# sjtuyinjie/Ground-Fusion2

Hardware: AMD Instinct MI355X
Metric: sliding-window solves/sec (10-kf, 2k landmarks) (higher is better)
Workload: dtype f64; 1 GPU; BASELINE configs[1]: 10-keyframe VI-wheel window, 2000 landmarks (K=9457 visual factors avg), marginalisation prior n=86, full optimization() = <=8 dogleg iterations + re-anchor + MARGIN_OLD; windows_per_gpu=8192, unique_windows=8, parallelism=windows sharded over 1 rank(s), no collective

## Files before the change

ground-fusion2_amd/csrc/gfbe_kernels.hip:

```cpp
#include "gfbe_devutil.h"
#include "gfbe_factors.h"
#include "gfbe_gnss_item.h"
#include <type_traits>

namespace gfd {

#ifndef GFBE_ASM_U
#define GFBE_ASM_U 4
#endif
#if GFBE_DIAG
#define ASM_TP_ON(d) (!(d).asm_legacy)
#else
#define ASM_TP_ON(d) true
#endif
#ifndef GFBE_KVIS_WAVES
#define GFBE_KVIS_WAVES 3
#endif
#ifndef GFBE_KVIS_STAMP
#define GFBE_KVIS_STAMP 0
#endif

#define PREP_WSYNC() do { __threadfence_block(); __builtin_amdgcn_wave_barrier(); } while (0)
template <int n>
__device__ __forceinline__ int sqrt_info_from_cov_wave(const double *cov, double *lu, double *inv, double *U, const int lane) {
// ... 594 lines not shown
          if (MODE != 1) {
            Hll += vc[u][1];
            gl += vc[u][2];
            if (YM) {
#pragma unroll
              for (int q = 0; q < 3; q++) Dsum[q] += vc[u][3 + q];
            } else {
#pragma unroll
              for (int q = 0; q < 6; q++) { hC[q] += vc[u][3 + q]; if (FULL) hC[6 + q] += vc[u][9 + q]; }
              if (FULL) hC[12] += vc[u][15];
            }
          }
        }
      }
    }
#undef VC_LD
    asm volatile("" :: "v"(cost));
    LSTAMP_ANY(18);
  }
  if (YM) {
#pragma unroll
    for (int q = 0; q < 3; q++) { hC[q] = Dsum[q]; hC[3 + q] = yx[q]; }
  }
  if (MODE == 0 && d.spec && tile == 0 && lane == 0) d.ctl[w].sw_mu[SPEC ? 1 - c.lb : c.lb] = SPEC ? mu_after_accept(c.mu) : c.mu;
  if (MODE == 0 && valid) {
    const bool first = !SPEC && c.iter == 0;
    const double mu_w = SPEC ? mu_after_accept(c.mu) : c.mu;
    double sl = 1.0, sw = 0.0;
    if (m > 0 && !is_const) {
      sl = first ? (d.opt.jacobi_scaling ? 1.0 / (1.0 + sqrt(Hll)) : 1.0) : d.lm_sl[slot];
      const double hs2 = sl * sl * Hll;
      sw = sqrt(sl * sl / (hs2 + mu_w * clamp_diag(hs2)));
    }
    if (first) d.lm_sl[slot] = sl;
    d.lm_sw[slot] = sw;
  }
  if (MODE != 1 && valid) {
    d.lm_Hll[slot] = Hll;
    d.lm_gl[slot] = gl;
#pragma unroll
    for (int q = 0; q < NHC; q++) d.lm_hC[(size_t)q * TL + slot] = hC[q];
  }
  KSTAMP(30);
  LSTAMP_ANY(19);
  cost = wave_sum(cost);
  if (lane == 0) {
    if (CAND) d.tile_cand[((size_t)w * d.max_tiles + tile) * 4] = cost;
    else d.tile_cost[(size_t)w * d.max_tiles + tile] = cost;
  }
}

__device__ __forceinline__ double candidate_tile(const BatchDev &d, const WinDesc &ds, const WinCtl &c, const int w, const int tile, const int t);
template <int MODE, bool FULL, bool SPEC = false>
__global__ __launch_bounds__(LM_TILE, (MODE == 0 && !FULL) ? GFBE_KVIS_WAVES : 2) void k_vis(BatchDev d0, int write_records) {
  const BatchDev d = MODE == 0 ? lin_view(d0, SPEC ? 1 - d0.ctl[blockIdx.x].lb : d0.ctl[blockIdx.x].lb) : d0;
  vis_body<MODE, FULL, 1, SPEC>(d, (MODE == 1 || SPEC) ? 0 : write_records, blockIdx.x, blockIdx.y, 0, (MODE == 1 || SPEC) && write_records);
}

#ifndef VIS_CHUNK
#define VIS_CHUNK 4
#endif
template <bool SPEC>
__global__ __launch_bounds__(LM_TILE, GFBE_KVIS_WAVES) void k_vis_chunk(BatchDev d0, int head_in, int nsub) {
  const int w = blockIdx.x;
  const WinCtl &c = d0.ctl[w];
  if (!SPEC && (c.done || c.reuse)) return;
  if (SPEC && (c.done || !c.have_step)) return;
  const int lbw = SPEC ? 1 - c.lb : c.lb;
  const BatchDev d = lin_view(d0, lbw);
  const WinDesc &ds = d.desc[w];
  const int sframe = blockIdx.y / nsub, sub = blockIdx.y - sframe * nsub;
  const int t0 = ds.sf_tile_begin[sframe] + VIS_CHUNK * sub, t1 = min(t0 + VIS_CHUNK, ds.sf_tile_begin[sframe + 1]);
  if (t0 >= t1) return;
  const int cur = c.cur, buf = SPEC ? 1 - cur : cur;
  const double *X = d.x + ((size_t)w * 2 + buf) * NA;
  const bool chead = SPEC && head_in;
  const double c1 = c.c1, c2 = c.c2;
  const bool first = !SPEC && c.iter == 0;
  const double mu_w = SPEC ? mu_after_accept(c.mu) : c.mu;
  const double sq = d.opt.vis_sqrt_info, delta = d.opt.huber_delta;
  const int jac_scale = d.opt.jacobi_scaling;
  const int lm_off_c = ds.lm_off;
  constexpr int XLD = 17;
  __shared__ PairConstY pcs[NF];
  __shared__ FrameConst fcs;
  __shared__ double xs[LM_TILE * XLD];
  const int lane = threadIdx.x;
  const size_t TL = d.tot_lm;
  int p_info;
  double p_pt[3], p_lam, p_sl = 0.0, p_vl = 0.0, p_yl = 0.0, p_ob[2];
#define VC_PREFETCH(TILE)                                                                                           \
  {                                                                                                                  \
    const int slot_ = lm_off_c + (TILE) * LM_TILE + lane;                                                            \
    p_info = d.lm_info[slot_];                                                                                       \
    _Pragma("unroll") for (int q = 0; q < 3; q++) p_pt[q] = d.lm_pts[(size_t)q * TL + slot_];                        \
    p_lam = d.lam[(size_t)(chead ? cur : buf) * TL + slot_];                                                         \
    if (chead) { p_sl = d.lm_sl[slot_]; p_vl = d.lm_vl[slot_]; p_yl = d.lm_yl[slot_]; }                              \
    p_ob[0] = d.lm_obs[slot_]; p_ob[1] = d.lm_obs[TL + slot_];                                                       \
  }
  VC_PREFETCH(t0)
  const double td = X[A_TD];
  {
    const double *src = d.pc + (((size_t)w * 3 + buf) * NPAIR + sframe * NF) * PC_DOUBLES;
    static_assert(PCY_DOUBLES <= LM_TILE && FC_DOUBLES <= LM_TILE, "one lane per entry of a pair record");
    const int ql = min(lane, (int)PCY_DOUBLES - 1);
    double rec[NF - 1];
#pragma unroll
    for (int jj = 0; jj < NF - 1; jj++) rec[jj] = src[(size_t)min(sframe + 1 + jj, NF - 1) * PC_DOUBLES + ql];
    const double fcv = src[(size_t)sframe * PC_DOUBLES + min(lane, (int)FC_DOUBLES - 1)];
#pragma unroll
    for (int jj = 0; jj < NF - 1; jj++) if (sframe + 1 + jj < NF && lane < (int)PCY_DOUBLES) ((double *)&pcs[min(sframe + 1 + jj, NF - 1)])[lane] = rec[jj];
    if (lane < (int)FC_DOUBLES) ((double *)&fcs)[lane] = fcv;
  }
  __syncthreads();
  for (int tile = t0; tile < t1; tile++) {
    const int slot = lm_off_c + tile * LM_TILE + lane;
    const int info = p_info;
    const double pix = p_pt[0], piy = p_pt[1], piz = p_pt[2];
    double lam = p_lam;
    const double c_sl = p_sl, c_vl = p_vl, c_yl = p_yl;
    double nob[2] = {p_ob[0], p_ob[1]};
    if (tile + 1 < t1) VC_PREFETCH(tile + 1)
    const bool valid = (info >> 24) & 1;
    const int m = valid ? ((info >> 8) & 0xff) : 0;
    const bool is_const = (info >> 16) & 1;
    int mmax = m;
#pragma unroll
    for (int o = 32; o > 0; o >>= 1) mmax = max(mmax, __shfl_xor(mmax, o, 64));
    double cost = 0.0;
    if (chead) {
      double d2, n2;
      lam = candidate_lm(lam, c_sl, c_vl, c_yl, c1, c2, valid && !is_const && m > 0, d2, n2);
      d.lam[(size_t)(1 - cur) * TL + slot] = lam;
      d2 = wave_sum(d2); n2 = wave_sum(n2);
      if (lane == 0) {
        double *o = d.tile_cand + ((size_t)w * d.max_tiles + tile) * 4;
        o[1] = d2; o[2] = n2;
      }
    }
    double Hll = 0.0, gl = 0.0, Dsum[3] = {0.0, 0.0, 0.0};
    const double yinv_l = 1.0 / lam;
    const double ycx = pix * yinv_l, ycy = piy * yinv_l, ycz = piz * yinv_l;
    vec3 yf, ye, yx;
#pragma unroll
    for (int a = 0; a < 3; a++) {
      yf[a] = __builtin_fma(fcs.W(a, 0), ycx, __builtin_fma(fcs.W(a, 1), ycy, fcs.W(a, 2) * ycz));
      ye[a] = yf[a] + fcs.wt[a];
      yx[a] = ye[a] + fcs.dPc[a];
    }
    double *xr = xs + lane * XLD;
    xr[7] = 0.0; xr[15] = 0.0;
    for (int k = 0; k < mmax; k++) {
      double r[2], Jl[2], hp[3];
      const double pjx = nob[0], pjy = nob[1];
      if (k + 1 < mmax) {
        const double *ob = d.lm_obs + (size_t)(k + 1) * 5 * TL + slot;
        nob[0] = ob[0]; nob[1] = ob[TL];
      }
      if (k < m) {
        double g0[3], g1[3];
        const double ck = visual_lin_y(pcs[sframe + 1 + k], ycx, ycy, ycz, yf, yinv_l, td, pjx, pjy, 0.0, 0.0, td, sq, delta, r, g0, g1, Jl);
        cost += ck;
        const vec3 y0 = cross3(mk3(g0[0], g0[1], g0[2]), yx), y1 = cross3(mk3(g1[0], g1[1], g1[2]), yx);
        const double w0 = is_const ? 0.0 : Jl[0], w1 = is_const ? 0.0 : Jl[1];
        vec3 dv;
#pragma unroll
        for (int q = 0; q < 3; q++) dv[q] = __builtin_fma(g0[q], w0, g1[q] * w1);
        Hll += __builtin_fma(w0, w0, w1 * w1);
        gl += __builtin_fma(w0, r[0], w1 * r[1]);
#pragma unroll
        for (int q = 0; q < 3; q++) Dsum[q] += dv[q];
#pragma unroll
        for (int q = 0; q < 3; q++) hp[q] = dv[q];
#pragma unroll
        for (int q = 0; q < 3; q++) { xr[q] = g0[q]; xr[3 + q] = y0[q]; xr[8 + q] = g1[q]; xr[11 + q] = y1[q]; }
        xr[6] = r[0]; xr[14] = r[1];
      } else {
#pragma unroll
        for (int q = 0; q < 7; q++) { xr[q] = 0.0; xr[8 + q] = 0.0; }
      }
#pragma unroll
      for (int q = 0; q < 2; q++) asm volatile("" : "+v"(nob[q]));
      if (k < m) {
#pragma unroll
        for (int q = 0; q < 3; q++) d.lm_hP[((size_t)k * 6 + q) * TL + slot] = hp[q];
      }
      typedef double dbl4_y __attribute__((ext_vector_type(4)));
      dbl4_y acc0 = {0, 0, 0, 0};
      const int lr = lane & 15, lk = lane >> 4;
      __threadfence_block();
      __builtin_amdgcn_wave_barrier();
#pragma unroll
      for (int blk = 0; blk < LM_TILE / 4 / 8; blk++) {
        double va[8];
#pragma unroll
        for (int u = 0; u < 8; u++) va[u] = xs[(4 * (8 * blk + u) + lk) * XLD + lr];
#pragma unroll
        for (int u = 0; u < 8; u++) acc0 = __builtin_amdgcn_mfma_f64_16x16x4f64(va[u], va[u], acc0, 0, 0, 0);
      }
      __builtin_amdgcn_wave_barrier();
      const double s0 = acc0[0] + __shfl_down(acc0[2], 8, 64), s1 = acc0[1] + __shfl_down(acc0[3], 8, 64);
      double *vo = d.vis_part + (((size_t)w * d.max_tiles + tile) * MAXOBS + k) * VPY_STRIDE;
      if (lr < 7) {
        { const int a = lk; if (a <= lr) vo[7 * a - a * (a - 1) / 2 + lr - a] = s0; }
        { const int a = lk + 4; if (a <= lr) vo[7 * a - a * (a - 1) / 2 + lr - a] = s1; }
      }
      __builtin_amdgcn_wave_barrier();
    }
    if (d.spec && tile == 0 && lane == 0) d.ctl[w].sw_mu[lbw] = mu_w;
    if (valid) {
      double sl = 1.0, sw = 0.0;
      if (m > 0 && !is_const) {
        sl = first ? (jac_scale ? 1.0 / (1.0 + sqrt(Hll)) : 1.0) : (chead ? c_sl : d.lm_sl[slot]);
        const double hs2 = sl * sl * Hll;
        sw = sqrt(sl * sl / (hs2 + mu_w * clamp_diag(hs2)));
      }
      if (first) d.lm_sl[slot] = sl;
      d.lm_sw[slot] = sw;
      d.lm_Hll[slot] = Hll;
      d.lm_gl[slot] = gl;
#pragma unroll
      for (int q = 0; q < 3; q++) { d.lm_hC[(size_t)q * TL + slot] = Dsum[q]; d.lm_hC[(size_t)(3 + q) * TL + slot] = yx[q]; }
    }
    cost = wave_sum(cost);
    if (lane == 0) {
      if (SPEC) d.tile_cand[((size_t)w * d.max_tiles + tile) * 4] = cost;
      else d.tile_cost[(size_t)w * d.max_tiles + tile] = cost;
    }
  }
#undef VC_PREFETCH
}

template <int MODE, bool FULL>
__global__ __launch_bounds__(LM_TILE, 1) void k_vis_split(BatchDev d, int write_records) {
  vis_body<MODE, FULL, LIN_SMALL_KS>(d, write_records, blockIdx.x, blockIdx.y / LIN_SMALL_KS, blockIdx.y % LIN_SMALL_KS);
}

template <int MODE>
__global__ __launch_bounds__(256) void k_lio_window(BatchDev d0, int spec) {
  const int w = blockIdx.y, wg = blockIdx.x, t = threadIdx.x;
  const WinDesc &ds = d0.desc[w];
  if (ds.lio_n == 0) return;
  const WinCtl &c = d0.ctl[w];
  if (MODE == 0 && !spec && (c.done || c.reuse)) return;
  if ((MODE == 1 || spec) && (c.done || !c.have_step)) return;
  const BatchDev d = MODE == 0 ? lin_view(d0, spec ? 1 - c.lb : c.lb) : d0;
  const int buf = (MODE == 1 || spec) ? 1 - c.cur : c.cur;
  const double *X = d.x + ((size_t)w * 2 + buf) * NA + A_POSE(ds.lio_frame);
  const vec3 tw = ld3(X);
  const mat3 R = qrot(ldq(X + 3));
  constexpr int NACC = (MODE == 0) ? 28 : 1;
  double acc[NACC];
#pragma unroll
  for (int q = 0; q < NACC; q++) acc[q] = 0.0;
  const double sq = ds.lio_sqrt_info, delta = ds.lio_huber;
  for (int k = wg * 256 + t; k < ds.lio_n; k += LIOW_WGS * 256) {
    const double *f = d.lio + (size_t)(ds.lio_off + k) * 8;
    const vec3 p = ld3(f), nv = ld3(f + 3);
    const double sw = sq * f[7];
    double r = sw * (dot3(nv, add(mv(R, p), tw)) + f[6]);
    double scale = 1.0, cost = 0.5 * r * r;
    if (delta > 0.0) {
      double s1, rs, asn;
      cost = corrector(r * r, delta, &s1, &rs, &asn);
      scale = s1;
    }
    if (MODE == 1) { acc[0] += cost; continue; }
    const vec3 nR = tmv(R, nv);
    double J[6];
    J[0] = sw * nv[0]; J[1] = sw * nv[1]; J[2] = sw * nv[2];
    J[3] = -sw * (nR[1] * p[2] - nR[2] * p[1]); J[4] = -sw * (nR[2] * p[0] - nR[0] * p[2]); J[5] = -sw * (nR[0] * p[1] - nR[1] * p[0]);
#pragma unroll
    for (int a = 0; a < 6; a++) J[a] *= scale;
    r *= scale;
    int e = 0;
#pragma unroll
    for (int a = 0; a < 6; a++)
#pragma unroll
      for (int b = a; b < 6; b++) acc[e++] += J[a] * J[b];
#pragma unroll
    for (int a = 0; a < 6; a++) acc[21 + a] += J[a] * r;
    acc[27] += cost;
  }
  __shared__ double red[4][NACC];
  const int lane = t & 63, wave = t >> 6;
#pragma unroll
  for (int q = 0; q < NACC; q++) {
    double v = acc[q];
#pragma unroll
    for (int o = 32; o > 0; o >>= 1) v += __shfl_xor(v, o, 64);
    if (lane == 0) red[wave][q] = v;
  }
  __syncthreads();
  double *out = d.lio_part + ((size_t)w * LIOW_WGS + wg) * LIOW_PART;
  if (t < NACC) out[MODE == 1 ? 28 : t] = red[0][t] + red[1][t] + red[2][t] + red[3][t];
}

__device__ __forceinline__ void pairsum_body(const BatchDev &d, const int marg, const int w, const int pair) {
  const WinDesc &ds = d.desc[w];
  const WinCtl &c = d.ctl[w];
  if (!marg && (c.done || c.reuse)) return;
  int i = 0, rem = pair;
  while (rem >= NF - 1 - i) { rem -= NF - 1 - i; i++; }
  const int j = i + 1 + rem;
  if (marg && i != 0) return;
  const int p = i * NF + j;
  if (ds.pair_begin[p + 1] == ds.pair_begin[p]) return;
  const double *vp = d.vis_part + (size_t)w * d.max_tiles * MAXOBS * VP_STRIDE + (size_t)(j - i - 1) * VP_STRIDE + threadIdx.x;
  double s = 0.0;
  for (int t = ds.sf_tile_begin[i]; t < ds.sf_tile_begin[i + 1]; t++) {
    if (((d.lm_info[ds.lm_off + t * LM_TILE] >> 8) & 0xff) <= j - i - 1) break;
    if (TILE_OWNED(d, t)) s += vp[(size_t)t * MAXOBS * VP_STRIDE];
  }
  if (marg) d.pair_part[((size_t)w * NF + j) * VP_STRIDE + threadIdx.x] = s;
}
__global__ __launch_bounds__(VP_STRIDE) void k_pairsum(BatchDev d, int marg) { pairsum_body(d, marg, blockIdx.y, blockIdx.x); }

__device__ __forceinline__ bool imu_nz(int r, int c) {
  const int mask[5] = {0x03F, 0x052, 0x09E, 0x108, 0x210};
  return (mask[r / 3] >> (c / 3)) & 1;
}
__device__ __forceinline__ bool wheel_nz(int r, int c) {
  if (c >= 20) return true;
  if (c >= 18) return r < 3;
  return r < 3 || ((c / 3) & 1);
}
__device__ __forceinline__ bool dense_pass_active(const WinCtl &c, int mode, int spec = 0) {
  if (mode == 0 && !spec && (c.done || c.reuse)) return false;
  if ((mode == 1 || spec) && (c.done || !c.have_step)) return false;
  return true;
}
#define RAW_IMU (15 + 15 * 30)
#define RAW_WHEEL (6 + 6 * 22)
__device__ __forceinline__ size_t raw_of(int f, int w, int B, int raw_len) { return ((size_t)f * ((B + 3) >> 2) + (w >> 2)) * raw_len * 4 + (w & 3); }
__global__ __launch_bounds__(64) void k_dense_raw(BatchDev d, int mode, int spec) {
  const int f = blockIdx.x, w = blockIdx.y * 64 + threadIdx.x;
  if (w >= d.B) return;
  const WinDesc &ds = d.desc[w];
  const WinCtl &c = d.ctl[w];
  if (!dense_pass_active(c, mode, spec)) return;
  const int buf = (mode == 1 || spec) ? 1 - c.cur : c.cur;
  const double *X = (mode >= 2) ? d.xout + (size_t)w * NA : d.x + ((size_t)w * 2 + buf) * NA;
  const size_t B = d.B;
  if (f < MAX_IMU) {
    if (f >= ds.n_imu) return;
    const int fi = ds.imu_frame[f];
    if (mode >= 2 && !(mode == 2 && fi == 0 && d.imu[ds.imu_off + f].sum_dt < 10.0)) return;
    double *out = d.raw_imu + raw_of(f, w, (int)B, RAW_IMU);
    imu_raw(&d.imu[ds.imu_off + f], d.opt.g_norm, X + A_POSE(fi), X + A_SB(fi), X + A_POSE(fi + 1), X + A_SB(fi + 1), out,
            mode == 1 ? nullptr : out + 15 * 4, 4);
  } else {
// ... 482 lines not shown
  } else {
    dense_body<true>(d, VM, 0, w, y - ny_tiles, SPEC, lsm);
  }
#if GFBE_LIN_STAMP
  if (MODE == GFBE_LIN_STAMP_MODE && (threadIdx.x & 63) == 0) {
    const int f = y - ny_tiles;
    const int kind = tile_wg ? 1 : (f < MAX_IMU ? 2 : (f < MAX_IMU + MAX_WHEEL ? 3 : (f == MAX_IMU + MAX_WHEEL ? 4 : 5)));
    atomicMax(ls + kind, (unsigned long long)wall_clock64());
    if (tile_wg && y == 0) ls[6] = wall_clock64();
    if (tile_wg && y == ny_tiles - 1) ls[7] = wall_clock64();
    if (threadIdx.x == 0 && f == MAX_IMU) ls[11] = wall_clock64();
  }
#endif
  if ((MODE == 1 || SPEC) && (fuse & 4)) {
    if (!tile_wg) { __syncthreads(); if (threadIdx.x >= 64) return; }
    WinCtl &c = d.ctl[w];
    AcceptLocal la;
    la.done = c.done; la.have_step = c.have_step; la.iter = c.iter; la.cur = c.cur; la.num_successful = c.num_successful;
    la.termination = c.termination; la.status = c.status; la.reuse = c.reuse; la.lb = c.lb;
    la.cost = c.cost; la.x_norm = c.x_norm; la.model_change = c.model_change; la.radius = c.radius; la.step_norm = c.step_norm; la.mu = c.mu;
    la.cand_cost = c.cand_cost;
    if (!arrive_last(d.win_cnt + 2 * w + 1, gridDim.y, threadIdx.x)) return;
#if GFBE_LIN_STAMP
    if (MODE == GFBE_LIN_STAMP_MODE && threadIdx.x == 0) ls[12] = wall_clock64();
#endif
    accept_body(d, w, threadIdx.x, la, c, SPEC ? 2 : 1);
    if (threadIdx.x == 0) {
      if (SPEC) c.lb = la.lb;
      c.done = la.done; c.have_step = la.have_step; c.cur = la.cur; c.num_successful = la.num_successful; c.termination = la.termination;
      c.status = la.status; c.reuse = la.reuse; c.cost = la.cost; c.x_norm = la.x_norm; c.radius = la.radius; c.mu = la.mu; c.cand_cost = la.cand_cost;
#if GFBE_LIN_STAMP
      if (MODE == GFBE_LIN_STAMP_MODE) ls[13] = wall_clock64();
#endif
    }
  }
}

typedef double dbl4_t __attribute__((ext_vector_type(4)));
#ifndef HS_LD
#define HS_LD 75
#endif

__device__ __forceinline__ int schur_pair(int I, int J) { return I * 5 - I * (I - 1) / 2 + (J - I); }

__device__ __forceinline__ int schur_group_first(int g, int ng) { return ng >= NF ? g : (g == 0 ? 0 : (g == 1 ? 2 : (g == 2 ? 3 : 6))); }
struct SchurLds {
  double hs[LM_TILE * HS_LD + 8];
  double s_rt[NF][12];
  int s_sf[NF + 1];
};
__device__ __forceinline__ SchurLds &schur_lds() { __shared__ SchurLds s; return s; }
template <bool LEAN>
__device__ __forceinline__ void schur_body(const BatchDev &d, const int marg, const int w, const int grp) {
  const WinDesc &ds = d.desc[w];
  WinCtl &c = d.ctl[w];
  if (!marg && (c.done || c.reuse)) return;
  if (marg && grp != 0) return;
  const int sub = (!marg && d.schur_groups == 2 * NF) ? 2 : 1;
  const int ng = marg ? NF : d.schur_groups / sub, half = grp % sub;
  const int gi = grp / sub;
  const int s_first = schur_group_first(gi, ng), s_end = marg ? 1 : (gi == ng - 1 ? NF : schur_group_first(gi + 1, ng));
  const int tb = ds.sf_tile_begin[s_first], te = ds.sf_tile_begin[s_end];
  const int tfirst = sub == 2 ? tb + half : tb + ((d.rank - tb) % d.world + d.world) % d.world;
  if (tfirst >= te) {
    if (marg) for (int q = threadIdx.x; q < SCHUR_STRIDE; q += 256) d.schur_part[((size_t)w * d.schur_groups) * SCHUR_STRIDE + q] = 0.0;
    return;
  }
  SchurLds &lds_ = schur_lds();
  double *const hs = lds_.hs;
  const size_t TL = d.tot_lm;
  const int t = threadIdx.x, lane = t & 63, wave = t >> 6;
  const bool compact = !marg;
  const int coff = compact ? 1 - 6 * s_first : 0;
  const int I0 = compact ? 0 : (6 * s_first) / 16;
  const int wv = __builtin_amdgcn_readfirstlane(wave);
  const int nside = compact ? (1 + 6 * (NF - s_first) + (d.vis_full ? 7 : 0) + 15) / 16 : 5 - I0, npairs = nside * (nside + 1) / 2;
  int pI[4], pJ[4];
#pragma unroll
  for (int q = 0; q < 4; q++) {
    int idx = 4 * q + wv, I = I0;
    pI[q] = -1; pJ[q] = -1;
    if (idx < npairs) {
      if (compact) { int J = 0; while ((J + 1) * (J + 2) / 2 <= idx) J++; pJ[q] = J; pI[q] = idx - J * (J + 1) / 2; }
      else { while (idx >= 5 - I) { idx -= 5 - I; I++; } pI[q] = I; pJ[q] = I + idx; }
    }
  }
  dbl4_t acc0 = {0.0, 0.0, 0.0, 0.0}, acc1 = acc0, acc2 = acc0, acc3 = acc0;
  const int lr = lane & 15, lk = lane >> 4;
  const int l = t & 63, part = t >> 6;
  const bool spec_sw = !marg && d.spec && c.sw_mu[c.lb] != c.mu;
  const double spec_mu = spec_sw ? c.mu : 0.0;
  const bool hc_full = !LEAN && (marg || d.vis_full);
  int *const s_sf = lds_.s_sf;
  double (*const s_rt)[12] = lds_.s_rt;
  const bool yrows = LEAN || (!marg && !d.vis_full);
  if (t <= NF) s_sf[t] = ds.sf_tile_begin[t];
  if (yrows && t < NF * 12) s_rt[t / 12][t % 12] = d.pc[(((size_t)w * 3 + c.cur) * NPAIR + (t / 12) * (NF + 1)) * PC_DOUBLES + LM_RT_OFF + t % 12];
  const int lm_off_c = ds.lm_off;
  __syncthreads();
  auto sframe_of = [&](int tile) __attribute__((always_inline)) { int sf = s_first; for (int q = s_first + 1; q < s_end; q++) sf += (tile >= s_sf[q]) ? 1 : 0; return sf; };
#define SCHUR_PV 20
#define SCHUR_PV_LEAN 12
#define SCHUR_PREFETCH(PV, PHLL, PSL, PINFO, PS, TILE)                                                                 \
  {                                                                                                                      \
    const int tile_ = min((TILE), te - 1);                                                                               \
    const int slot_ = lm_off_c + tile_ * LM_TILE + l;                                                                    \
    PS = sframe_of(tile_);                                                                                               \
    const int klast_ = max(NF - 2 - PS, 0);                     \
    PINFO = d.lm_info[slot_];                                                                                            \
    PHLL = (marg || spec_sw ? d.lm_Hll : d.lm_sw)[slot_];               \
    if (spec_sw) PSL = d.lm_sl[slot_];                  \
    const double *gl_ = d.lm_gl + slot_;                                                                                 \
     \
     \
    if (LEAN) {                                                                                                          \
      _Pragma("unroll") for (int idx_ = 0; idx_ < SCHUR_PV_LEAN; idx_++) {                                                 \
        const int u_ = max(idx_ - 3, 0) / 3, q_ = max(idx_ - 3, 0) - 3 * u_;                                             \
        const int kk_ = min(part - 1 + 3 * u_, klast_), k9_ = min(9, klast_);                                            \
        const double *src_ = idx_ < 3 ? d.lm_hC + (size_t)(3 + idx_) * TL + slot_                                       \
                           : (part == 0 ? (u_ == 0 ? d.lm_hC + (size_t)q_ * TL + slot_                                  \
                                                   : (u_ == 1 ? gl_ : d.lm_hP + ((size_t)k9_ * 6 + q_) * TL + slot_))   \
                                        : d.lm_hP + ((size_t)kk_ * 6 + q_) * TL + slot_);                                \
        PV[idx_] = *src_;                                                                                                \
      }                                                                                                                  \
    } else                                                                                                               \
    _Pragma("unroll") for (int idx_ = 0; idx_ < SCHUR_PV; idx_++) {                                                      \
      const int u_ = idx_ / 6, q_ = idx_ - 6 * u_;                                                                       \
      const int kk_ = min(part - 1 + 3 * u_, klast_), k9_ = min(9, klast_);                                              \
       \
      const int q9_ = idx_ - HC - 1;                                                                                     \
      const double *src_ = part == 0 ? (idx_ < HC ? d.lm_hC + (size_t)((idx_ < 6 || hc_full) ? idx_ : 5) * TL + slot_   \
                                                  : (idx_ == HC ? gl_ : ((yrows && q9_ >= 3) ? d.lm_hC + (size_t)q9_ * TL + slot_ \
                                                                                             : d.lm_hP + ((size_t)k9_ * 6 + q9_) * TL + slot_))) \
                                     : ((yrows && q_ >= 3) ? d.lm_hC + (size_t)q_ * TL + slot_ : d.lm_hP + ((size_t)kk_ * 6 + q_) * TL + slot_); \
      PV[idx_] = *src_;                                                                                                  \
    }                                                                                                                    \
  }
  const bool stamp_wg = (w == 0 && grp == 0 && t == 0 && !marg);
  double *stamp = d.timing + 8;
  if (stamp_wg) { stamp[0] = (double)wall_clock64(); stamp[5] = (double)clock64(); }
  const int tstep = sub == 2 ? 2 : d.world;
#define SCHUR_SLOT(Q, ACC)                                                                          \
    if (pI[Q] >= 0 && (compact ? pJ[Q] <= jl : ((pI[Q] <= jl || pI[Q] == 4) && (pJ[Q] <= jl || pJ[Q] == 4)))) {   \
      const double *pa = hs + 16 * pI[Q] + lr + lk * HS_LD, *pb = hs + 16 * pJ[Q] + lr + lk * HS_LD; \
      _Pragma("unroll") for (int hf = 0; hf < 2; hf++) {       \
        double va[LM_TILE / 8], vb[LM_TILE / 8];                                                    \
        _Pragma("unroll") for (int kk = 0; kk < LM_TILE / 8; kk++) { va[kk] = pa[4 * (8 * hf + kk) * HS_LD]; vb[kk] = pb[4 * (8 * hf + kk) * HS_LD]; } \
        _Pragma("unroll") for (int kk = 0; kk < LM_TILE / 8; kk++) ACC = __builtin_amdgcn_mfma_f64_16x16x4f64(va[kk], vb[kk], ACC, 0, 0, 0); \
      }                                                                                             \
    }
#define SCHUR_LEAN_SLOT(Q, ACC)                                                                                        \
    if (pI[Q] >= 0 && pJ[Q] <= jl) {                                                                                     \
      const double *pa = hs + 16 * pI[Q] + lr + lk * HS_LD, *pb = hs + 16 * pJ[Q] + lr + lk * HS_LD;                     \
      _Pragma("unroll") for (int c_ = 0; c_ < 4; c_++) if (4 * c_ < nk) {                                                \
        double va[4], vb[4];                                                                                             \
        _Pragma("unroll") for (int kk = 0; kk < 4; kk++) { va[kk] = pa[4 * (4 * c_ + kk) * HS_LD]; vb[kk] = pb[4 * (4 * c_ + kk) * HS_LD]; } \
        _Pragma("unroll") for (int kk = 0; kk < 4; kk++) ACC = __builtin_amdgcn_mfma_f64_16x16x4f64(va[kk], vb[kk], ACC, 0, 0, 0); \
      }                                                                                                                  \
    }
#define SCHUR_RUN_TILE(PV, PHLL, PSL, PINFO, PS, TILE, REFILL)                                                          \
  {                                                                                                                      \
    __syncthreads();                                                                                                     \
    if (stamp_wg && (TILE) == tfirst) stamp[1] = (double)wall_clock64();                                                 \
    const int ps = PS, pm0 = __builtin_amdgcn_readfirstlane(PINFO);                                                      \
    const int jl = __builtin_amdgcn_readfirstlane(compact ? (d.vis_full ? nside - 1 : (6 * (ps - s_first + ((pm0 >> 8) & 0xff) + 1)) >> 4) \
                                                          : (6 * (ps + ((pm0 >> 8) & 0xff) + 1) - 1) >> 4);              \
     \
    const unsigned long long vmask_ = LEAN ? __builtin_amdgcn_ballot_w64((PINFO >> 24) & 1) : ~0ull;                       \
    const int nk = vmask_ ? (64 - __builtin_clzll(vmask_) + 3) >> 2 : 0;                                                 \
    {                                                                                                                    \
      const int s = ps, kmax = NF - 1 - s;                                                  \
      const bool valid = (PINFO >> 24) & 1;                                                                              \
      const int m = (PINFO >> 8) & 0xff;                                                                                 \
      const bool is_const = (PINFO >> 16) & 1;                                                                           \
      double sw = 0.0;                                                                                                   \
      if (valid && m > 0 && (marg || !is_const))                                                                         \
        sw = marg ? sqrt((PHLL > d.opt.marg_eps) ? 1.0 / PHLL : 0.0) : PHLL;                                             \
      if (spec_sw && valid && m > 0 && !is_const) {                    \
        const double hs2_ = PSL * PSL * PHLL;                                                                            \
        sw = sqrt(PSL * PSL / (hs2_ + spec_mu * clamp_diag(hs2_)));                                                      \
      }                                                                                                                  \
      double *row = hs + l * HS_LD + coff;                                                                               \
      if (part == 0) {                                                                                                   \
        for (int q = compact ? 6 * s_first : 16 * I0; q < 6 * s; q++) row[q] = 0.0;                                      \
        double blk0[6];                                                                                                  \
        if (yrows) lm_row_block(s_rt[s], PV + (LEAN ? 3 : 0), PV + (LEAN ? 0 : 3), true, blk0);                      \
        else { _Pragma("unroll") for (int q = 0; q < 6; q++) blk0[q] = PV[q]; }                                          \
        _Pragma("unroll") for (int q = 0; q < 6; q++) { row[6 * s + q] = sw * blk0[q]; row[T_EX + q] = hc_full ? sw * PV[6 + q] : 0.0; } \
        row[T_TD] = hc_full ? sw * PV[12] : 0.0;                                                                         \
        if (compact) {                                                                                                   \
          row[-coff] = sw * PV[LEAN ? 6 : HC];                                                 \
          for (int q = NV + coff; q < min(16 * nside, (int)HS_LD); q++) row[q - coff] = 0.0;      \
        } else {                                                                                                         \
          row[NV] = sw * PV[HC];                                                                                         \
          _Pragma("unroll") for (int q = NV + 1; q < HS_LD; q++) row[q] = 0.0;                                           \
        }                                                                                                                \
        if (9 < kmax) {                                                    \
          const bool written = valid && 9 < m;                                                                           \
          double blk9[6];                                                                                                \
          if (yrows) lm_row_block(s_rt[min(s + 10, NF - 1)], PV + (LEAN ? 9 : HC + 1), PV + (LEAN ? 0 : 3), false, blk9);                       \
          else { _Pragma("unroll") for (int q = 0; q < 6; q++) blk9[q] = PV[HC + 1 + q]; }                               \
          _Pragma("unroll") for (int q = 0; q < 6; q++) row[6 * (s + 10) + q] = written ? sw * blk9[q] : 0.0;            \
        }                                                                                                                \
      } else {                                                                                                           \
        _Pragma("unroll") for (int u = 0; u < 3; u++) {                                                                  \
          const int k = part - 1 + 3 * u;                                                                                \
          if (k < kmax) {                                                                                                \
             \
            const bool written = valid && k < m;                                                                         \
            double blkk[6];                                                                                              \
            if (yrows) lm_row_block(s_rt[s + 1 + k], PV + (LEAN ? 3 + 3 * u : 6 * u), PV + (LEAN ? 0 : 6 * u + 3), false, blkk);     \
            else { _Pragma("unroll") for (int q = 0; q < 6; q++) blkk[q] = PV[u * 6 + q]; }                              \
            _Pragma("unroll") for (int q = 0; q < 6; q++) row[6 * (s + 1 + k) + q] = written ? sw * blkk[q] : 0.0;       \
          }                                                                                                              \
        }                                                                                                                \
      }                                                                                                                  \
    }                                                                                                                    \
    __syncthreads();                                                                                                     \
    if (stamp_wg && (TILE) == tfirst) stamp[2] = (double)wall_clock64();                                                 \
    SCHUR_PREFETCH(PV, PHLL, PSL, PINFO, PS, (REFILL))          \
    if (LEAN) {                                                                                                         \
      SCHUR_LEAN_SLOT(0, acc0) SCHUR_LEAN_SLOT(1, acc1) SCHUR_LEAN_SLOT(2, acc2) SCHUR_LEAN_SLOT(3, acc3)               \
    } else {                                                                                                             \
      SCHUR_SLOT(0, acc0)                                                                                                \
      SCHUR_SLOT(1, acc1)                                                                                                \
      SCHUR_SLOT(2, acc2)                                                                                                \
      SCHUR_SLOT(3, acc3)                                                                                                \
    }                                                                                                                    \
  }
  double preA[SCHUR_PV], aHll = 0.0, aSl = 0.0;
  int aInfo = 0, aS = 0;
  SCHUR_PREFETCH(preA, aHll, aSl, aInfo, aS, tfirst)
  for (int tile = tfirst; tile < te; tile += tstep) SCHUR_RUN_TILE(preA, aHll, aSl, aInfo, aS, tile, tile + tstep)
#undef SCHUR_RUN_TILE
#undef SCHUR_SLOT
#undef SCHUR_LEAN_SLOT
#undef SCHUR_PREFETCH
#undef SCHUR_PV
#undef SCHUR_PV_LEAN
  if (stamp_wg) { stamp[3] = (double)wall_clock64(); stamp[4] = (double)(te - tb); stamp[6] = (double)clock64(); }
  double *out = d.schur_part + ((size_t)w * d.schur_groups + grp) * SCHUR_STRIDE;
#define SCHUR_OUT(Q, ACC)                                                         \
  if (pI[Q] >= 0) {                                                               \
    double *o = out + (size_t)(compact ? pJ[Q] * (pJ[Q] + 1) / 2 + pI[Q] : schur_pair(pI[Q], pJ[Q])) * 256; \
    _Pragma("unroll") for (int r = 0; r < 4; r++) o[(lk + 4 * r) * 16 + lr] = ACC[r]; \
  }
  SCHUR_OUT(0, acc0)
  SCHUR_OUT(1, acc1)
  SCHUR_OUT(2, acc2)
  SCHUR_OUT(3, acc3)
#undef SCHUR_OUT
}
#ifndef GFBE_SCHUR_WGS
#define GFBE_SCHUR_WGS 4
#endif
__global__ __launch_bounds__(256, GFBE_SCHUR_WGS) void k_schur(BatchDev d0, int marg) {
  const BatchDev d = marg ? d0 : lin_view(d0, d0.ctl[blockIdx.x].lb);
  if (!marg && d.schur_groups == SCHUR_GROUPS && !d.vis_full) schur_body<true>(d, 0, blockIdx.x, blockIdx.y);
  else schur_body<false>(d, marg, blockIdx.x, blockIdx.y);
}
#ifndef GFBE_LINSCHUR_WGS
#define GFBE_LINSCHUR_WGS 3
#endif
#define LS_XLD 17
template <bool SPEC>
__global__ __launch_bounds__(256, GFBE_LINSCHUR_WGS) void k_linschur(BatchDev d0, int head_in, int gate_mu) {
  const int w = blockIdx.x;
  const int grp = blockIdx.y == 1 ? 2 : (blockIdx.y == 2 ? 1 : (int)blockIdx.y);
  const WinCtl &c = d0.ctl[w];
  if (c.done) return;
  if (SPEC) { if (!c.have_step) return; }
  else { if (c.reuse) return; if (gate_mu && c.sw_mu[c.lb] == c.mu) return; }
  const int lbw = SPEC ? 1 - c.lb : c.lb;
  const BatchDev d = lin_view(d0, lbw);
  const WinDesc &ds = d.desc[w];
  const int s_first = schur_group_first(grp, SCHUR_GROUPS), s_end = grp == SCHUR_GROUPS - 1 ? (int)NF : schur_group_first(grp + 1, SCHUR_GROUPS);
  const int tb = ds.sf_tile_begin[s_first], te = ds.sf_tile_begin[s_end];
  if (tb >= te) return;
  __shared__ double hs[LM_TILE * HS_LD + 8];
  static_assert(4 * LM_TILE * LS_XLD <= LM_TILE * HS_LD + 8, "the evaluation panels live inside the Schur panel");
  __shared__ double Psum[4][5][LM_TILE];
  __shared__ double Pcost[4];
  __shared__ PairConstY pcs[NF];
  __shared__ FrameConst fcs;
  __shared__ double s_rt[NF][12];
  const int t = threadIdx.x, lane = t & 63, wave = t >> 6;
  const int wv = __builtin_amdgcn_readfirstlane(wave);
  const int rot = __builtin_amdgcn_readfirstlane((int)(((unsigned)w * 0x9E3779B1u) >> 20) + grp);
  const int mr = (wv + rot) & 3;
  const size_t TL = d.tot_lm;
  const int cur = c.cur;
  const int buf = SPEC ? 1 - cur : cur;
  const double *X = d.x + ((size_t)w * 2 + buf) * NA;
  const double *pcw = d.pc + ((size_t)w * 3 + buf) * NPAIR * PC_DOUBLES;
  const bool chead = SPEC && head_in;
  const double c1 = c.c1, c2 = c.c2;
  const bool first = !SPEC && c.iter == 0;
  const double mu_w = SPEC ? mu_after_accept(c.mu) : c.mu;
  const double sq = d.opt.vis_sqrt_info, delta = d.opt.huber_delta;
  const int jac_scale = d.opt.jacobi_scaling;
  const double td = X[A_TD];
  int sfb[NF + 1];
#pragma unroll
  for (int q = 0; q <= NF; q++) sfb[q] = ds.sf_tile_begin[q];
  const int lm_off_c = ds.lm_off;
  if (t < NF * 12) s_rt[t / 12][t % 12] = pcw[(size_t)(t / 12) * (NF + 1) * PC_DOUBLES + LM_RT_OFF + t % 12];
  const int coff = 1 - 6 * s_first;
  const int nside = (1 + 6 * (NF - s_first) + 15) / 16, npairs = nside * (nside + 1) / 2;
  int pI[4], pJ[4];
#pragma unroll
  for (int q = 0; q < 4; q++) {
    const int idx = 4 * q + mr;
    pI[q] = -1; pJ[q] = -1;
    if (idx < npairs) { int J = 0; while ((J + 1) * (J + 2) / 2 <= idx) J++; pJ[q] = J; pI[q] = idx - J * (J + 1) / 2; }
  }
  dbl4_t acc0 = {0.0, 0.0, 0.0, 0.0}, acc1 = acc0, acc2 = acc0, acc3 = acc0;
  const int lr = lane & 15, lk = lane >> 4;
  double *const xs = hs + (size_t)wave * (LM_TILE * LS_XLD);
  int p_info;
  double p_pt[3], p_lam, p_sl = 1.0, p_vl = 0.0, p_yl = 0.0, p_ob[3][2];
#define LS_PREFETCH(TILE)                                                                                           \
  {                                                                                                                  \
    const int er_ = (wv + rot + (TILE)) & 3;                                                                         \
    const int tile_ = min((TILE), te - 1);                                                                           \
    const int slot_ = lm_off_c + tile_ * LM_TILE + lane;                                                             \
    p_info = d.lm_info[slot_];                                                                                       \
    _Pragma("unroll") for (int q = 0; q < 3; q++) p_pt[q] = d.lm_pts[(size_t)q * TL + slot_];                        \
    p_lam = d.lam[(size_t)(chead ? cur : buf) * TL + slot_];                                                         \
    if (chead) { p_vl = d.lm_vl[slot_]; p_yl = d.lm_yl[slot_]; }                                                     \
    if (!first) p_sl = d.lm_sl[slot_];                                                                               \
    _Pragma("unroll") for (int u = 0; u < 3; u++) {                                                                  \
      const int k_ = min(er_ + 4 * u, (int)MAXOBS - 1);                                                              \
      p_ob[u][0] = d.lm_obs[((size_t)k_ * 5 + 0) * TL + slot_];                                                      \
      p_ob[u][1] = d.lm_obs[((size_t)k_ * 5 + 1) * TL + slot_];                                                      \
    }                                                                                                                \
  }
  LS_PREFETCH(tb)
  int cur_sf = -1;
  for (int tile = tb; tile < te; tile++) {
    int sf = s_first;
#pragma unroll
    for (int q = 1; q < NF; q++) sf += (q > s_first && q < s_end && tile >= sfb[q]) ? 1 : 0;
    if (sf != cur_sf) {
      const double *src = pcw + (size_t)sf * NF * PC_DOUBLES;
      for (int e = t; e < (NF - 1 - sf) * (int)PCY_DOUBLES; e += 256) {
        const int j = sf + 1 + e / (int)PCY_DOUBLES, q = e % (int)PCY_DOUBLES;
        ((double *)&pcs[j])[q] = src[(size_t)j * PC_DOUBLES + q];
      }
      if (t < (int)FC_DOUBLES) ((double *)&fcs)[t] = src[(size_t)sf * PC_DOUBLES + t];
      cur_sf = sf;
    }
    __syncthreads();
    const int er = (wv + rot + tile) & 3;
    const int slot = lm_off_c + tile * LM_TILE + lane;
    const int info = p_info;
    const bool valid = (info >> 24) & 1;
    const int m = valid ? ((info >> 8) & 0xff) : 0;
    const bool is_const = (info >> 16) & 1;
    int mmax = m;
#pragma unroll
    for (int o = 32; o > 0; o >>= 1) mmax = max(mmax, __shfl_xor(mmax, o, 64));
    mmax = __builtin_amdgcn_readfirstlane(mmax);
    double lam = p_lam;
    const double sl_old = p_sl;
    if (chead) {
      double d2, n2;
      lam = candidate_lm(lam, sl_old, p_vl, p_yl, c1, c2, valid && !is_const && m > 0, d2, n2);
      if (er == 0) {
        d.lam[(size_t)(1 - cur) * TL + slot] = lam;
        d2 = wave_sum(d2); n2 = wave_sum(n2);
        if (lane == 0) { double *o = d.tile_cand + ((size_t)w * d.max_tiles + tile) * 4; o[1] = d2; o[2] = n2; }
      }
    }
    const double yinv_l = 1.0 / lam;
    const double ycx = p_pt[0] * yinv_l, ycy = p_pt[1] * yinv_l, ycz = p_pt[2] * yinv_l;
    vec3 yf, yx;
#pragma unroll
    for (int a = 0; a < 3; a++) {
      yf[a] = __builtin_fma(fcs.W(a, 0), ycx, __builtin_fma(fcs.W(a, 1), ycy, fcs.W(a, 2) * ycz));
      yx[a] = (yf[a] + fcs.wt[a]) + fcs.dPc[a];
    }
    double *xr = xs + lane * LS_XLD;
    xr[7] = 0.0; xr[15] = 0.0;
    double Hq = 0.0, gq = 0.0, Dq[3] = {0.0, 0.0, 0.0}, cq = 0.0, dk[3][3];
// ... 1938 lines not shown
```

Before: 129,600 solves/s.

## Skip empty MFMA blocks and redundant row zeroing in landmark and Schur kernels

In the landmark linearisation kernel, a wave ballot over active observations sets how many 16-lane groups hold data. The per-observation MFMA outer-product loop only runs over those groups, and the zero-fill is limited to lanes inside them. In the Schur tile builder, a per-16-row chunk bound (jlc) skips MFMA chunks whose column block lies past that chunk's extent. Row zeroing for the pose prefix and the extrinsic/TD/tail columns is done only when the frame index changes or on the first tile, and observation blocks past the tile's minimum count are zeroed instead of being computed. This cuts wasted MFMA and shared-memory traffic on sparse tiles, at the cost of extra branching, a non-unrolled loop, and correctness depending on LDS rows staying valid between tiles.

```diff
diff --git a/ground-fusion2_amd/csrc/gfbe_kernels.hip b/ground-fusion2_amd/csrc/gfbe_kernels.hip
--- a/ground-fusion2_amd/csrc/gfbe_kernels.hip
+++ b/ground-fusion2_amd/csrc/gfbe_kernels.hip
@@ -770,6 +770,8 @@
     xr[7] = 0.0; xr[15] = 0.0;
     for (int k = 0; k < mmax; k++) {
       double r[2], Jl[2], hp[3];
+      const unsigned long long act = __builtin_amdgcn_ballot_w64(k < m);
+      const int ng = act ? (64 - __builtin_clzll(act) + 15) >> 4 : 0;
       const double pjx = nob[0], pjy = nob[1];
       if (k + 1 < mmax) {
         const double *ob = d.lm_obs + (size_t)(k + 1) * 5 * TL + slot;
@@ -793,7 +795,7 @@
 #pragma unroll
         for (int q = 0; q < 3; q++) { xr[q] = g0[q]; xr[3 + q] = y0[q]; xr[8 + q] = g1[q]; xr[11 + q] = y1[q]; }
         xr[6] = r[0]; xr[14] = r[1];
-      } else {
+      } else if (lane < 16 * ng) {
 #pragma unroll
         for (int q = 0; q < 7; q++) { xr[q] = 0.0; xr[8 + q] = 0.0; }
       }
@@ -808,13 +810,13 @@
       const int lr = lane & 15, lk = lane >> 4;
       __threadfence_block();
       __builtin_amdgcn_wave_barrier();
-#pragma unroll
-      for (int blk = 0; blk < LM_TILE / 4 / 8; blk++) {
-        double va[8];
-#pragma unroll
-        for (int u = 0; u < 8; u++) va[u] = xs[(4 * (8 * blk + u) + lk) * XLD + lr];
-#pragma unroll
-        for (int u = 0; u < 8; u++) acc0 = __builtin_amdgcn_mfma_f64_16x16x4f64(va[u], va[u], acc0, 0, 0, 0);
+#pragma unroll 1
+      for (int blk = 0; blk < ng; blk++) {
+        double va[4];
+#pragma unroll
+        for (int u = 0; u < 4; u++) va[u] = xs[(4 * (4 * blk + u) + lk) * XLD + lr];
+#pragma unroll
+        for (int u = 0; u < 4; u++) acc0 = __builtin_amdgcn_mfma_f64_16x16x4f64(va[u], va[u], acc0, 0, 0, 0);
       }
       __builtin_amdgcn_wave_barrier();
       const double s0 = acc0[0] + __shfl_down(acc0[2], 8, 64), s1 = acc0[1] + __shfl_down(acc0[3], 8, 64);
@@ -1603,7 +1605,7 @@
 #define SCHUR_LEAN_SLOT(Q, ACC)                                                                                        \
     if (pI[Q] >= 0 && pJ[Q] <= jl) {                                                                                     \
       const double *pa = hs + 16 * pI[Q] + lr + lk * HS_LD, *pb = hs + 16 * pJ[Q] + lr + lk * HS_LD;                     \
-      _Pragma("unroll") for (int c_ = 0; c_ < 4; c_++) if (4 * c_ < nk) {                                                \
+      _Pragma("unroll") for (int c_ = 0; c_ < 4; c_++) if (4 * c_ < nk && pJ[Q] <= jlc[c_]) {                            \
         double va[4], vb[4];                                                                                             \
         _Pragma("unroll") for (int kk = 0; kk < 4; kk++) { va[kk] = pa[4 * (4 * c_ + kk) * HS_LD]; vb[kk] = pb[4 * (4 * c_ + kk) * HS_LD]; } \
         _Pragma("unroll") for (int kk = 0; kk < 4; kk++) ACC = __builtin_amdgcn_mfma_f64_16x16x4f64(va[kk], vb[kk], ACC, 0, 0, 0); \
@@ -1613,12 +1615,21 @@
   {                                                                                                                      \
     __syncthreads();                                                                                                     \
     if (stamp_wg && (TILE) == tfirst) stamp[1] = (double)wall_clock64();                                                 \
-    const int ps = PS, pm0 = __builtin_amdgcn_readfirstlane(PINFO);                                                      \
+    const int ps = __builtin_amdgcn_readfirstlane(PS), pm0 = __builtin_amdgcn_readfirstlane(PINFO);                      \
     const int jl = __builtin_amdgcn_readfirstlane(compact ? (d.vis_full ? nside - 1 : (6 * (ps - s_first + ((pm0 >> 8) & 0xff) + 1)) >> 4) \
                                                           : (6 * (ps + ((pm0 >> 8) & 0xff) + 1) - 1) >> 4);              \
      \
     const unsigned long long vmask_ = LEAN ? __builtin_amdgcn_ballot_w64((PINFO >> 24) & 1) : ~0ull;                       \
     const int nk = vmask_ ? (64 - __builtin_clzll(vmask_) + 3) >> 2 : 0;                                                 \
+     \
+     \
+     \
+    int jlc[4];                                                                                                          \
+    _Pragma("unroll") for (int c_ = 0; c_ < 4; c_++)                                                                     \
+      jlc[c_] = LEAN ? (6 * (ps - s_first + ((__builtin_amdgcn_readlane(PINFO, 16 * c_) >> 8) & 0xff) + 1)) >> 4 : jl; \
+    const int m0_ = (pm0 >> 8) & 0xff, lim_ = 16 * (jl + 1) - coff;                                                      \
+    const bool first_ = !LEAN || prev_s < 0, fresh_ = !LEAN || ps != prev_s;                                             \
+    prev_s = ps;                                                                                                         \
     {                                                                                                                    \
       const int s = ps, kmax = NF - 1 - s;                                                  \
       const bool valid = (PINFO >> 24) & 1;                                                                              \
@@ -1633,20 +1644,26 @@
       }                                                                                                                  \
       double *row = hs + l * HS_LD + coff;                                                                               \
       if (part == 0) {                                                                                                   \
-        for (int q = compact ? 6 * s_first : 16 * I0; q < 6 * s; q++) row[q] = 0.0;                                      \
+         \
+        if (fresh_) for (int q = compact ? 6 * s_first : 16 * I0; q < 6 * s; q++) row[q] = 0.0;                          \
         double blk0[6];                                                                                                  \
         if (yrows) lm_row_block(s_rt[s], PV + (LEAN ? 3 : 0), PV + (LEAN ? 0 : 3), true, blk0);                      \
         else { _Pragma("unroll") for (int q = 0; q < 6; q++) blk0[q] = PV[q]; }                                          \
-        _Pragma("unroll") for (int q = 0; q < 6; q++) { row[6 * s + q] = sw * blk0[q]; row[T_EX + q] = hc_full ? sw * PV[6 + q] : 0.0; } \
-        row[T_TD] = hc_full ? sw * PV[12] : 0.0;                                                                         \
+        _Pragma("unroll") for (int q = 0; q < 6; q++) row[6 * s + q] = sw * blk0[q];                                     \
+        if (first_) {                                                                                                    \
+          _Pragma("unroll") for (int q = 0; q < 6; q++) row[T_EX + q] = hc_full ? sw * PV[6 + q] : 0.0;                  \
+          row[T_TD] = hc_full ? sw * PV[12] : 0.0;                                                                       \
+        }                                                                                                                \
         if (compact) {                                                                                                   \
           row[-coff] = sw * PV[LEAN ? 6 : HC];                                                 \
-          for (int q = NV + coff; q < min(16 * nside, (int)HS_LD); q++) row[q - coff] = 0.0;      \
+          if (first_) for (int q = NV + coff; q < min(16 * nside, (int)HS_LD); q++) row[q - coff] = 0.0;      \
         } else {                                                                                                         \
           row[NV] = sw * PV[HC];                                                                                         \
           _Pragma("unroll") for (int q = NV + 1; q < HS_LD; q++) row[q] = 0.0;                                           \
         }                                                                                                                \
-        if (9 < kmax) {                                                    \
+        if (9 < kmax && LEAN && m0_ <= 9) {                               \
+          _Pragma("unroll") for (int q = 0; q < 6; q++) if (6 * (s + 10) + q < lim_) row[6 * (s + 10) + q] = 0.0;        \
+        } else if (9 < kmax) {                                             \
           const bool written = valid && 9 < m;                                                                           \
           double blk9[6];                                                                                                \
           if (yrows) lm_row_block(s_rt[min(s + 10, NF - 1)], PV + (LEAN ? 9 : HC + 1), PV + (LEAN ? 0 : 3), false, blk9);                       \
@@ -1655,8 +1672,10 @@
         }                                                                                                                \
       } else {                                                                                                           \
         _Pragma("unroll") for (int u = 0; u < 3; u++) {                                                                  \
-          const int k = part - 1 + 3 * u;                                                                                \
-          if (k < kmax) {                                                                                                \
+          const int k = (LEAN ? wv : part) - 1 + 3 * u;                                                                  \
+          if (k < kmax && LEAN && k >= m0_) {                                                                            \
+            _Pragma("unroll") for (int q = 0; q < 6; q++) if (6 * (s + 1 + k) + q < lim_) row[6 * (s + 1 + k) + q] = 0.0; \
+          } else if (k < kmax) {                                                                                         \
              \
             const bool written = valid && k < m;                                                                         \
             double blkk[6];                                                                                              \
@@ -1681,6 +1700,7 @@
   }
   double preA[SCHUR_PV], aHll = 0.0, aSl = 0.0;
   int aInfo = 0, aS = 0;
+  int prev_s = -1;
   SCHUR_PREFETCH(preA, aHll, aSl, aInfo, aS, tfirst)
   for (int tile = tfirst; tile < te; tile += tstep) SCHUR_RUN_TILE(preA, aHll, aSl, aInfo, aS, tile, tile + tstep)
 #undef SCHUR_RUN_TILE
```

Result: no change. 131,500 solves/s, median of 6 (+1.5%).
